# uoguelph-mlrg/Theano-MPI

Hardware: NVIDIA H100
Metric: AlexNet-128b BSP seconds per 5120 images (train+comm, device-timed, max over ranks) (lower is better)
Workload: dtype bf16; 1 GPU; model=AlexNet, global_batch=128, input=3x227x227, parallelism=dp1, rule=BSP, push_master=False, cuda_graph=True, overlap=True

## Files before the change

### theanompi_b200/csrc/api.h

```cpp
#pragma once
#include <cuda_runtime.h>
#include <stdint.h>
#include "common.cuh"

namespace tmpi {

constexpr int kMaxRanks = 8;
constexpr int kMaxCommBlocks = 1024;

struct CommCtx {
  void* arena[kMaxRanks];
  uint32_t* sig[kMaxRanks];
  uint32_t* epoch;
  void* mc_arena;
  int rank, world;
  long long spin_limit;
};

struct FusedArgs {
  CommCtx ctx;
  long long w_off, g_off, u_off, h_off, wire_off;
  const uint8_t* block_group;
  GroupTable tab;
  const float* lr_ptr;
  float mu;
// ... 2 lines not shown
  long long lo, hi;
  int wire16;
  int pre_reduced;
  int push_master = 1;
};

struct ReduceArgs {
  CommCtx ctx;
  long long src_off, dst_off, h_off;
  const uint8_t* block_group;
  GroupTable tab;
  float scale;
  long long lo, hi;
  int skip_local_groups;
};

void gemm_set_debug(int flags);
void gemm_set_bulk(int mask);
void gemm_rs_configure(int world, const void* const* peer_g , const void* local_g);
void gemm_rs_add_range(const void* c_lo, const void* c_hi, long long blo, long long per);
void gemm_rs_clear();
int gemm_plan_splits(int tiles, int num_kb, int sms);
int gemm_plan_tall(long long M, int nt, int out_bf16, int sms);
void gemm(const void* A, const void* B, void* C, const float* bias, int M, int N, int K, long long lda, long long ldb, long long ldc,
          int a_mn, int b_mn, int out_bf16, int bias_mode, int relu, float alpha, int bn_hint, int splitk, int f32, cudaStream_t st);
void gemm_sgd(const void* A, const void* B, void* W, void* U, void* H, const void* lr_ptr, float lr_mult, float wd, float mu, int nesterov,
              float inv_k, int M, int N, int K, long long lda, long long ldb, long long ldw, int f32, cudaStream_t st);

void conv_fprop(const void* x, const void* w, void* y, const float* bias, int N, int H, int W, int Ctot, int c_off, int Cg, int KH,
                int KW, int Ho, int Wo, int S, int P, int O, long long ldc, int relu, int dgrad, int f32, cudaStream_t st);
void conv_wgrad(const void* dy, const void* x, void* dw, int N, int H, int W, int Ctot, int c_off, int Cg, int KH, int KW, int Ho,
                int Wo, int S, int P, int O, long long ldy, int f32, cudaStream_t st);
void conv_fprop2(const void* x, const void* w0, const void* w1, void* y0, void* y1, const float* bias0, const float* bias1, int N, int H,
                 int W, int Ctot, int c_off0, int c_off1, int Cg, int KH, int KW, int Ho, int Wo, int S, int P, int O, long long ldc,
                 int relu, int dgrad, int f32, cudaStream_t st);
void conv_wgrad2(const void* dy0, const void* dy1, const void* x, void* dw0, void* dw1, int N, int H, int W, int Ctot, int c_off0,
                 int c_off1, int Cg, int KH, int KW, int Ho, int Wo, int S, int P, int O, long long ldy, int f32, cudaStream_t st);

void space_to_depth(const void* x, void* y, int N, int H, int W, int C, int S, int Hs, int Ws, int Cp, int P, int f32, cudaStream_t st);
void s2d_filter(const void* src, void* dst, int O, int KH, int KW, int C, int S, int KHs, int KWs, int Cp, int dir, int f32, cudaStream_t st);
void lrn_fwd(const void* x, void* y, long long rows, int C, int n, float k, float alpha, float beta, int f32, cudaStream_t st);
void lrn_bwd(const void* x, const void* dy, void* dx, long long rows, int C, int n, float k, float alpha, float beta, int f32, cudaStream_t st);
void pool_fwd(const void* x, void* y, void* arg, int N, int H, int W, int C, int Ho, int Wo, int k, int s, int p, int is_max, int f32,
              cudaStream_t st);
void pool_bwd(const void* dy, const void* arg, void* dx, int N, int H, int W, int C, int Ho, int Wo, int k, int s, int p, int is_max, int f32,
              cudaStream_t st);
// ... 75 lines not shown
```

### theanompi_b200/csrc/binding.cpp

```cpp
#include <pybind11/pybind11.h>
#include <pybind11/stl.h>

#include <cstring>
#include <memory>
#include <vector>

#include "api.h"
#include "peer_arena.h"

namespace py = pybind11;
using namespace tmpi;
typedef uintptr_t ptr_t;

static inline void* P(ptr_t p) { return reinterpret_cast<void*>(p); }
static inline cudaStream_t S(ptr_t s) { return reinterpret_cast<cudaStream_t>(s); }

static GroupTable make_table(const std::vector<float>& lr_mult, const std::vector<float>& wd, const std::vector<int>& exch) {
  GroupTable t;
  for (int i = 0; i < kMaxGroups; ++i) {
    t.lr_mult[i] = i < (int)lr_mult.size() ? lr_mult[i] : 1.f;
    t.wd[i] = i < (int)wd.size() ? wd[i] : 0.f;
    t.exch[i] = i < (int)exch.size() ? exch[i] : 1;
  }
  return t;
// ... 2 lines not shown
struct PyComm {
  std::unique_ptr<PeerArena> pa;
};

PYBIND11_MODULE(_tmpi_native, m) {
  m.doc() = "theanompi_b200 native sm_90a kernels and peer-memory runtime";
  m.def("launch_count", [] { return (unsigned long long)g_launch_count.load(); });
  m.def("reset_launch_count", [] { g_launch_count.store(0); });
  m.def("capture_status", [](ptr_t st) {
    cudaStreamCaptureStatus s = cudaStreamCaptureStatusNone;
    cudaError_t e = cudaStreamIsCapturing(S(st), &s);
    return py::make_tuple((int)e, (int)s);
  });
  m.attr("ARENA_BLOCK") = kArenaBlock;
  m.attr("MAX_RANKS") = kMaxRanks;
  m.attr("MAX_COMM_BLOCKS") = kMaxCommBlocks;

  m.def("gemm_set_debug", &gemm_set_debug);
  m.def("gemm_set_bulk", &gemm_set_bulk);
  m.def("gemm_rs_add_range", [](ptr_t c_lo, ptr_t c_hi, long long blo, long long per) { gemm_rs_add_range(P(c_lo), P(c_hi), blo, per); });
  m.def("gemm_rs_clear", &gemm_rs_clear);
  m.def("gemm_plan_splits", &gemm_plan_splits);
  m.def("gemm_plan_tall", &gemm_plan_tall);
  m.def("gemm", [](ptr_t A, ptr_t B, ptr_t C, ptr_t bias, int M, int N, int K, long long lda, long long ldb, long long ldc, int a_mn, int b_mn,
                   int out_bf16, int bias_mode, int relu, float alpha, int bn_hint, int splitk, int f32, ptr_t st) {
    gemm(P(A), P(B), P(C), (const float*)P(bias), M, N, K, lda, ldb, ldc, a_mn, b_mn, out_bf16, bias_mode, relu, alpha, bn_hint, splitk, f32,
         S(st));
  }, py::arg("A"), py::arg("B"), py::arg("C"), py::arg("bias"), py::arg("M"), py::arg("N"), py::arg("K"), py::arg("lda"), py::arg("ldb"),
     py::arg("ldc"), py::arg("a_mn"), py::arg("b_mn"), py::arg("out_bf16"), py::arg("bias_mode"), py::arg("relu"), py::arg("alpha"),
     py::arg("bn_hint"), py::arg("splitk"), py::arg("f32"), py::arg("st"));
  m.def("gemm_sgd", [](ptr_t A, ptr_t B, ptr_t W, ptr_t U, ptr_t H, ptr_t lr_ptr, float lr_mult, float wd, float mu, int nesterov, float inv_k,
                       int M, int N, int K, long long lda, long long ldb, long long ldw, int f32, ptr_t st) {
    gemm_sgd(P(A), P(B), P(W), P(U), P(H), P(lr_ptr), lr_mult, wd, mu, nesterov, inv_k, M, N, K, lda, ldb, ldw, f32, S(st));
  }, py::arg("A"), py::arg("B"), py::arg("W"), py::arg("U"), py::arg("H"), py::arg("lr_ptr"), py::arg("lr_mult"), py::arg("wd"),
     py::arg("mu"), py::arg("nesterov"), py::arg("inv_k"), py::arg("M"), py::arg("N"), py::arg("K"), py::arg("lda"), py::arg("ldb"),
     py::arg("ldw"), py::arg("f32"), py::arg("st"));

  m.def("conv_fprop", [](ptr_t x, ptr_t w, ptr_t y, ptr_t bias, int N, int H, int W, int Ctot, int c_off, int Cg, int KH, int KW, int Ho, int Wo,
                         int Sd, int Pd, int O, long long ldc, int relu, int dgrad, int f32, ptr_t st) {
    conv_fprop(P(x), P(w), P(y), (const float*)P(bias), N, H, W, Ctot, c_off, Cg, KH, KW, Ho, Wo, Sd, Pd, O, ldc, relu, dgrad, f32, S(st)); });
  m.def("conv_wgrad", [](ptr_t dy, ptr_t x, ptr_t dw, int N, int H, int W, int Ctot, int c_off, int Cg, int KH, int KW, int Ho, int Wo, int Sd,
                         int Pd, int O, long long ldy, int f32, ptr_t st) {
    conv_wgrad(P(dy), P(x), P(dw), N, H, W, Ctot, c_off, Cg, KH, KW, Ho, Wo, Sd, Pd, O, ldy, f32, S(st)); });
  m.def("conv_fprop2", [](ptr_t x, ptr_t w0, ptr_t w1, ptr_t y0, ptr_t y1, ptr_t b0, ptr_t b1, int N, int H, int W, int Ctot, int c_off0, int c_off1,
                          int Cg, int KH, int KW, int Ho, int Wo, int Sd, int Pd, int O, long long ldc, int relu, int dgrad, int f32, ptr_t st) {
    conv_fprop2(P(x), P(w0), P(w1), P(y0), P(y1), (const float*)P(b0), (const float*)P(b1), N, H, W, Ctot, c_off0, c_off1, Cg, KH, KW, Ho, Wo,
// ... 165 lines not shown
```

### theanompi_b200/csrc/gemm_wgmma.cu

```cuda
#include "gemm_wgmma.cuh"
#include <vector>

namespace tmpi {
std::atomic<unsigned long long> g_launch_count{0};

namespace wgmma {

int g_dbg = 0;
int g_bulk = -1;

static int choose_splits(int tiles, int num_kb, int sms) {
  if (deterministic_mode()) return 1;
  if (tiles >= sms || num_kb < 8) return 1;
  const int kTileOverheadKb = 4;
  int best = 1;
  long long best_cost = -1;
  const int max_s = std::min(num_kb / 4, 4 * sms);
  for (int s = 1; s <= max_s; ++s) {
    const int kb_per = (num_kb + s - 1) / s;
    const int s_eff = (num_kb + kb_per - 1) / kb_per;
    const long long waves = ((long long)tiles * s_eff + sms - 1) / sms;
    const long long cost = waves * (kb_per + kTileOverheadKb) * 64 + s_eff;
    if (best_cost < 0 || cost < best_cost) { best_cost = cost; best = s_eff; }
  }
  return best;
}

static bool use_tall_tiles(long long M, int nt, int eligible, int sms) {
  static const bool enabled = [] { const char* e = getenv("TMPI_GEMM_TALL"); return !(e && e[0] == '0'); }();
  if (!enabled || !eligible || M < 2 * BM) return false;
  const long long t1 = ((M + BM - 1) / BM) * nt, t2 = ((M + 2 * BM - 1) / (2 * BM)) * nt;
  const long long w1 = (t1 + sms - 1) / sms, w2 = (t2 + sms - 1) / sms;
  return w2 * 17 <= w1 * 10;
}

}

void gemm_set_debug(int flags) { wgmma::g_dbg = flags; }
void gemm_set_bulk(int mask) { wgmma::g_bulk = mask; }

namespace wgmma {
struct RsRange { const char* lo; const char* hi; long long blo, per; };
static int g_rs_world = 0, g_rs_rank = 0;
static float* g_rs_peer[kMaxRanks] = {};
static const char* g_rs_local = nullptr;
static std::vector<RsRange> g_rs_ranges;
static std::mutex g_rs_mu;
static bool rs_lookup(const void* C, Params& p) {
  std::lock_guard<std::mutex> lk(g_rs_mu);
  if (g_rs_world < 2) return false;
  const char* c = reinterpret_cast<const char*>(C);
  for (const RsRange& r : g_rs_ranges) {
    if (c >= r.lo && c < r.hi) {
      p.rs_world = g_rs_world; p.rs_rank = g_rs_rank;
      p.rs_blo = (unsigned)r.blo; p.rs_per = (unsigned)std::max<long long>(1, r.per);
      p.rs_e0 = (long long)((c - g_rs_local) / 4);
// ... 8 lines not shown
void gemm_rs_configure(int world, const void* const* peer_g, const void* local_g) {
  std::lock_guard<std::mutex> lk(wgmma::g_rs_mu);
  if (world > kMaxRanks) throw std::runtime_error("gemm_rs_configure: too many ranks");
  wgmma::g_rs_world = world;
  wgmma::g_rs_local = reinterpret_cast<const char*>(local_g);
  wgmma::g_rs_rank = 0;
  for (int q = 0; q < world; ++q) {
    wgmma::g_rs_peer[q] = reinterpret_cast<float*>(const_cast<void*>(peer_g[q]));
    if (peer_g[q] == local_g) wgmma::g_rs_rank = q;
  }
  wgmma::g_rs_ranges.clear();
}
void gemm_rs_add_range(const void* c_lo, const void* c_hi, long long blo, long long per) {
  std::lock_guard<std::mutex> lk(wgmma::g_rs_mu);
  wgmma::g_rs_ranges.push_back({reinterpret_cast<const char*>(c_lo), reinterpret_cast<const char*>(c_hi), blo, per});
}
void gemm_rs_clear() {
  std::lock_guard<std::mutex> lk(wgmma::g_rs_mu);
  wgmma::g_rs_world = 0; wgmma::g_rs_ranges.clear();
}

int gemm_plan_splits(int tiles, int num_kb, int sms) { return wgmma::choose_splits(tiles, num_kb, sms); }
int gemm_plan_tall(long long M, int nt, int out_bf16, int sms) { return wgmma::use_tall_tiles(M, nt, out_bf16, sms) ? 1 : 0; }

namespace wgmma {
template <typename T>
static void gemm_host(const void* A, const void* B, void* C, const float* bias, int M, int N, int K, long long lda, long long ldb,
                      long long ldc, int a_mn, int b_mn, int out_bf16, int bias_mode, int relu, float alpha, int bn_hint, int splitk,
                      cudaStream_t st) {
  using E = Elem<T>;
  constexpr int BK = E::BK, ATOM = E::ATOM, ESZ = E::ESZ;
  if (M <= 0 || N <= 0 || K <= 0) return;
  const int sms = sm_count();
  const int mt = (M + BM - 1) / BM;
  const bool fused_epi = bias_mode != 0 || relu;
  const bool can_split = (!out_bf16) && !fused_epi;
  int BN = bn_hint;
  if (BN == 0) {
    BN = 128;
    if (!(can_split && splitk != 1)) {
      if (mt * ((N + 127) / 128) < sms && N >= 64) BN = 64;
      if (BN == 64 && mt * ((N + 63) / 64) < sms && !b_mn && N >= 32) BN = 32;
    } else if (N <= 64) {
      BN = 64;
    }
  }
// ... 99 lines not shown
  cuuint64_t dims[3] = {(cuuint64_t)Cg, (cuuint64_t)taps, (cuuint64_t)O};
  cuuint64_t strides[2] = {(cuuint64_t)Cg * esz, (cuuint64_t)taps * Cg * esz};
  cuuint32_t box[3] = {(cuuint32_t)box_c, 1u, (cuuint32_t)box_o};
  cuuint32_t estr[3] = {1u, 1u, 1u};
  CUresult r = get_encode()(&m, esz == 4 ? f32_map_type() : CU_TENSOR_MAP_DATA_TYPE_BFLOAT16, 3, const_cast<void*>(w), dims, strides,
                            box, estr, CU_TENSOR_MAP_INTERLEAVE_NONE, swz, CU_TENSOR_MAP_L2_PROMOTION_L2_256B,
                            CU_TENSOR_MAP_FLOAT_OOB_FILL_NONE);
  if (r != CUDA_SUCCESS) throw std::runtime_error("tmpi_native: cuTensorMapEncodeTiled(3D weights) failed, code " + std::to_string((int)r));
  if (cache.size() > 4096) cache.clear();
  cache[key] = m;
  return m;
}

template <typename T>
static void conv_fprop_groups(int ngroups, const void* x, const int* c_off, const void* const* w, void* const* y, const float* const* bias,
                              int N, int H, int W, int Ctot, int Cg, int KH, int KW, int Ho, int Wo, int S, int P, int O, long long ldc,
                              int relu, int out_bf16, int dgrad, cudaStream_t st) {
  using E = Elem<T>;
  constexpr int BK = E::BK, ATOM = E::ATOM, ESZ = E::ESZ;
  const long long M = (long long)N * Ho * Wo;
  if (M <= 0 || O <= 0) return;
  if (M >= (1LL << 31)) throw std::runtime_error("conv_fprop: too many output pixels");
  if (ESZ == 4) out_bf16 = 0;
  const int BN = O > 64 ? 128 : 64;
  Params p;
  p.C = y[0]; p.bias = bias[0]; p.alpha = 1.f; p.M = (int)M; p.N = O; p.K = KH * KW * Cg; p.ldc = ldc; p.a_mn = 0; p.b_mn = dgrad ? 1 : 0;
  p.groups = ngroups; p.C1 = ngroups > 1 ? y[1] : nullptr; p.bias1 = ngroups > 1 ? bias[1] : nullptr;
  p.out_bf16 = out_bf16; p.bias_mode = bias[0] ? 1 : 0; p.relu = relu; p.atomic_out = 0;
  if (ngroups > 1 && ((bias[0] == nullptr) != (bias[1] == nullptr))) throw std::runtime_error("conv_fprop: both groups need a bias or none");
  if (dgrad && (S != 1 || ((O * ESZ) % 16) != 0)) throw std::runtime_error("conv dgrad through the fprop kernel needs stride 1 and 16-byte channel rows");
  p.nt = (O + BN - 1) / BN; p.splits = 1;
  const bool tall = use_tall_tiles(M, p.nt * ngroups, ESZ == 2 ? out_bf16 : !dgrad, sm_count());
  p.mt = tall ? (int)((M + 2 * BM - 1) / (2 * BM)) : (int)((M + BM - 1) / BM);
  p.group_m = 0;
  p.conv_mode = 1; p.cHo = Ho; p.cWo = Wo; p.cS = S; p.cP = P; p.cKH = KH; p.cKW = KW; p.cCg = Cg; p.c_chunks = (Cg + BK - 1) / BK;
  p.num_kb = KH * KW * p.c_chunks; p.kb_per_split = p.num_kb;
  CUtensorMap ta[2], tb[2];
  for (int g = 0; g < ngroups; ++g) {
    ta[g] = make_im2col_map(x, N, H, W, Ctot, c_off[g], Cg, KH, KW, S, P, BM, ESZ, 0);
    tb[g] = dgrad ? make_weight_map(w[g], Cg, KH * KW, O, BK, ATOM, ESZ, 1) : make_weight_map(w[g], O, KH * KW, Cg, BN, BK, ESZ, 0);
  }
  const CUtensorMap* a1 = ngroups > 1 ? &ta[1] : nullptr;
  const CUtensorMap* b1 = ngroups > 1 ? &tb[1] : nullptr;
  if (tall) { if (BN == 128) launch<T, 128, 2>(ta[0], tb[0], p, 1, st, a1, b1); else launch<T, 64, 2>(ta[0], tb[0], p, 1, st, a1, b1); }
  else if (BN == 128) launch<T, 128, 1>(ta[0], tb[0], p, 1, st, a1, b1);
  else launch<T, 64, 1>(ta[0], tb[0], p, 1, st, a1, b1);
}

template <typename T>
static void conv_wgrad_groups(int ngroups, const void* const* dy, const void* x, void* const* dw, const int* c_off, int N, int H, int W,
                              int Ctot, int Cg, int KH, int KW, int Ho, int Wo, int S, int P, int O, long long ldy, cudaStream_t st) {
  using E = Elem<T>;
  constexpr int BK = E::BK, ATOM = E::ATOM, ESZ = E::ESZ;
  const long long M = (long long)N * Ho * Wo;
  if (M <= 0 || O <= 0) return;
  if (M >= (1LL << 31)) throw std::runtime_error("conv_wgrad: too many output pixels");
  const int sms = sm_count();
  const int BN = 128;
  Params p;
  p.C = dw[0]; p.bias = nullptr; p.alpha = 1.f; p.M = O; p.N = KH * KW * Cg; p.K = (int)M; p.ldc = (long long)KH * KW * Cg; p.a_mn = 1; p.b_mn = 1;
  p.groups = ngroups; p.C1 = ngroups > 1 ? dw[1] : nullptr; p.bias1 = nullptr;
  p.out_bf16 = 0; p.bias_mode = 0; p.relu = 0;
  p.group_m = 0;
  p.conv_mode = 2; p.cHo = Ho; p.cWo = Wo; p.cS = S; p.cP = P; p.cKH = KH; p.cKW = KW; p.cCg = Cg; p.c_chunks = (Cg + ATOM - 1) / ATOM;
  p.mt = (O + BM - 1) / BM; p.nt = (KH * KW * p.c_chunks + BN / ATOM - 1) / (BN / ATOM);
  p.num_kb = (int)((M + BK - 1) / BK);
  int splits = choose_splits(p.mt * p.nt * ngroups, p.num_kb, sms);
  p.kb_per_split = (p.num_kb + splits - 1) / splits;
  splits = (p.num_kb + p.kb_per_split - 1) / p.kb_per_split;
  p.splits = splits; p.atomic_out = splits > 1;
  CUtensorMap ta[2], tb[2];
  for (int g = 0; g < ngroups; ++g) {
    if (splits > 1) check_cuda(cudaMemsetAsync(dw[g], 0, (size_t)O * KH * KW * Cg * 4, st), "conv_wgrad memset");
    ta[g] = make_tmap(dy[g], (uint64_t)O, (uint64_t)M, (uint64_t)ldy * ESZ, (uint32_t)BK, ESZ, 1);
    tb[g] = make_im2col_map(x, N, H, W, Ctot, c_off[g], Cg, KH, KW, S, P, BK, ESZ, 1);
  }
  launch<T, 128, 1>(ta[0], tb[0], p, splits, st, ngroups > 1 ? &ta[1] : nullptr, ngroups > 1 ? &tb[1] : nullptr);
}
}

void conv_fprop(const void* x, const void* w, void* y, const float* bias, int N, int H, int W, int Ctot, int c_off, int Cg, int KH,
                int KW, int Ho, int Wo, int S, int P, int O, long long ldc, int relu, int dgrad, int f32, cudaStream_t st) {
  const void* ws[1] = {w}; void* ys[1] = {y}; const float* bs[1] = {bias};
  if (f32) wgmma::conv_fprop_groups<float>(1, x, &c_off, ws, ys, bs, N, H, W, Ctot, Cg, KH, KW, Ho, Wo, S, P, O, ldc, relu, 0, dgrad, st);
  else wgmma::conv_fprop_groups<__nv_bfloat16>(1, x, &c_off, ws, ys, bs, N, H, W, Ctot, Cg, KH, KW, Ho, Wo, S, P, O, ldc, relu, 1, dgrad, st);
}

void conv_fprop2(const void* x, const void* w0, const void* w1, void* y0, void* y1, const float* bias0, const float* bias1, int N, int H,
                 int W, int Ctot, int c_off0, int c_off1, int Cg, int KH, int KW, int Ho, int Wo, int S, int P, int O, long long ldc,
                 int relu, int dgrad, int f32, cudaStream_t st) {
  const int co[2] = {c_off0, c_off1}; const void* ws[2] = {w0, w1}; void* ys[2] = {y0, y1}; const float* bs[2] = {bias0, bias1};
  if (f32) wgmma::conv_fprop_groups<float>(2, x, co, ws, ys, bs, N, H, W, Ctot, Cg, KH, KW, Ho, Wo, S, P, O, ldc, relu, 0, dgrad, st);
  else wgmma::conv_fprop_groups<__nv_bfloat16>(2, x, co, ws, ys, bs, N, H, W, Ctot, Cg, KH, KW, Ho, Wo, S, P, O, ldc, relu, 1, dgrad, st);
}

void conv_wgrad(const void* dy, const void* x, void* dw, int N, int H, int W, int Ctot, int c_off, int Cg, int KH, int KW, int Ho,
                int Wo, int S, int P, int O, long long ldy, int f32, cudaStream_t st) {
  const void* dys[1] = {dy}; void* dws[1] = {dw};
  if (f32) wgmma::conv_wgrad_groups<float>(1, dys, x, dws, &c_off, N, H, W, Ctot, Cg, KH, KW, Ho, Wo, S, P, O, ldy, st);
  else wgmma::conv_wgrad_groups<__nv_bfloat16>(1, dys, x, dws, &c_off, N, H, W, Ctot, Cg, KH, KW, Ho, Wo, S, P, O, ldy, st);
// ... 11 lines not shown
```

### theanompi_b200/csrc/gemm_wgmma.cuh

```cuda
#pragma once
#include "common.cuh"
#include "api.h"
#include <cuda.h>
#include <algorithm>
#include <map>
#include <mutex>
#include <tuple>

namespace tmpi {

namespace wgmma {

constexpr int BM = 128;
constexpr int NUM_THREADS = 384;
constexpr int NUM_CONSUMER_WARPS = 8;
constexpr int PRODUCER_REGS = 40, CONSUMER_REGS = 232;

template <typename T> struct SgdEpilogue {};
template <typename OP> struct Operand { using Type = OP; static constexpr bool kSgd = false; };
template <typename T> struct Operand<SgdEpilogue<T>> { using Type = T; static constexpr bool kSgd = true; };

template <typename T> struct Elem {
  static constexpr int ESZ = (int)sizeof(T);
  static constexpr int BK = 128 / ESZ;
// ... 177 lines not shown
}

__device__ __forceinline__ void wgmma(float (&d)[16], uint64_t da, uint64_t db, uint32_t scale_d, WgTF32<32>) {
  asm volatile("{\n\t.reg .pred p;\n\tsetp.ne.b32 p, %18, 0;\n\t"
               "wgmma.mma_async.sync.aligned.m64n32k8.f32.tf32.tf32 {%0, %1, %2, %3, %4, %5, %6, %7, %8, %9, %10, %11, %12, %13, %14, %15}, %16, %17, p, 1, 1;\n\t}"
               : "+f"(d[0]), "+f"(d[1]), "+f"(d[2]), "+f"(d[3]), "+f"(d[4]), "+f"(d[5]), "+f"(d[6]), "+f"(d[7]), "+f"(d[8]), "+f"(d[9]), "+f"(d[10]), "+f"(d[11]), "+f"(d[12]), "+f"(d[13]), "+f"(d[14]), "+f"(d[15])
               : "l"(da), "l"(db), "r"(scale_d));
}

__device__ __forceinline__ void wgmma(float (&d)[32], uint64_t da, uint64_t db, uint32_t scale_d, WgTF32<64>) {
  asm volatile("{\n\t.reg .pred p;\n\tsetp.ne.b32 p, %34, 0;\n\t"
               "wgmma.mma_async.sync.aligned.m64n64k8.f32.tf32.tf32 {%0, %1, %2, %3, %4, %5, %6, %7, %8, %9, %10, %11, %12, %13, %14, %15, %16, %17, %18, %19, %20, %21, %22, %23, %24, %25, %26, %27, %28, %29, %30, %31}, %32, %33, p, 1, 1;\n\t}"
               : "+f"(d[0]), "+f"(d[1]), "+f"(d[2]), "+f"(d[3]), "+f"(d[4]), "+f"(d[5]), "+f"(d[6]), "+f"(d[7]), "+f"(d[8]), "+f"(d[9]), "+f"(d[10]), "+f"(d[11]), "+f"(d[12]), "+f"(d[13]), "+f"(d[14]), "+f"(d[15]), "+f"(d[16]), "+f"(d[17]), "+f"(d[18]), "+f"(d[19]), "+f"(d[20]), "+f"(d[21]), "+f"(d[22]), "+f"(d[23]), "+f"(d[24]), "+f"(d[25]), "+f"(d[26]), "+f"(d[27]), "+f"(d[28]), "+f"(d[29]), "+f"(d[30]), "+f"(d[31])
               : "l"(da), "l"(db), "r"(scale_d));
}

__device__ __forceinline__ void wgmma(float (&d)[64], uint64_t da, uint64_t db, uint32_t scale_d, WgTF32<128>) {
  asm volatile("{\n\t.reg .pred p;\n\tsetp.ne.b32 p, %66, 0;\n\t"
               "wgmma.mma_async.sync.aligned.m64n128k8.f32.tf32.tf32 {%0, %1, %2, %3, %4, %5, %6, %7, %8, %9, %10, %11, %12, %13, %14, %15, %16, %17, %18, %19, %20, %21, %22, %23, %24, %25, %26, %27, %28, %29, %30, %31, %32, %33, %34, %35, %36, %37, %38, %39, %40, %41, %42, %43, %44, %45, %46, %47, %48, %49, %50, %51, %52, %53, %54, %55, %56, %57, %58, %59, %60, %61, %62, %63}, %64, %65, p, 1, 1;\n\t}"
               : "+f"(d[0]), "+f"(d[1]), "+f"(d[2]), "+f"(d[3]), "+f"(d[4]), "+f"(d[5]), "+f"(d[6]), "+f"(d[7]), "+f"(d[8]), "+f"(d[9]), "+f"(d[10]), "+f"(d[11]), "+f"(d[12]), "+f"(d[13]), "+f"(d[14]), "+f"(d[15]), "+f"(d[16]), "+f"(d[17]), "+f"(d[18]), "+f"(d[19]), "+f"(d[20]), "+f"(d[21]), "+f"(d[22]), "+f"(d[23]), "+f"(d[24]), "+f"(d[25]), "+f"(d[26]), "+f"(d[27]), "+f"(d[28]), "+f"(d[29]), "+f"(d[30]), "+f"(d[31]), "+f"(d[32]), "+f"(d[33]), "+f"(d[34]), "+f"(d[35]), "+f"(d[36]), "+f"(d[37]), "+f"(d[38]), "+f"(d[39]), "+f"(d[40]), "+f"(d[41]), "+f"(d[42]), "+f"(d[43]), "+f"(d[44]), "+f"(d[45]), "+f"(d[46]), "+f"(d[47]), "+f"(d[48]), "+f"(d[49]), "+f"(d[50]), "+f"(d[51]), "+f"(d[52]), "+f"(d[53]), "+f"(d[54]), "+f"(d[55]), "+f"(d[56]), "+f"(d[57]), "+f"(d[58]), "+f"(d[59]), "+f"(d[60]), "+f"(d[61]), "+f"(d[62]), "+f"(d[63])
               : "l"(da), "l"(db), "r"(scale_d));
}

__device__ __forceinline__ uint64_t make_smem_desc(uint32_t smem_addr, uint32_t lbo_bytes, uint32_t sbo_bytes) {
  uint64_t d = 0;
  d |= (uint64_t)((smem_addr & 0x3FFFF) >> 4);
  d |= (uint64_t)((lbo_bytes >> 4) & 0x3FFF) << 16;
  d |= (uint64_t)((sbo_bytes >> 4) & 0x3FFF) << 32;
  d |= (uint64_t)1 << 62;
  return d;
}

template <typename T, int BN, int MT, int TA, int TB>
__device__ __forceinline__ void mma_kblock(float (&acc)[MT][BN / 2], uint64_t da, uint64_t db, uint32_t a_step, uint32_t b_step) {
  constexpr int STEPS = Elem<T>::BK / Elem<T>::MMA_K;
  constexpr uint64_t SUB = (uint64_t)(BM * 128) >> 4;
#pragma unroll
  for (int k = 0; k < STEPS; ++k) {
#pragma unroll
    for (int u = 0; u < MT; ++u) {
      if constexpr (Elem<T>::TF32) wgmma(acc[u], da + u * SUB + a_step * k, db + b_step * k, 1u, WgTF32<BN>{});
      else wgmma(acc[u], da + u * SUB + a_step * k, db + b_step * k, 1u, WgBF16<BN, TA, TB>{});
    }
  }
}

__device__ __forceinline__ void xpose_tf32(uint8_t* dst, const uint8_t* src, int rows, int tid) {
  for (int c = tid; c < rows * 8; c += 128) {
    const int k = c & 31, mn = (c >> 5) * 4;
    const int mi = mn & 31;
    const float4 v = *reinterpret_cast<const float4*>(src + (mn >> 5) * 4096 + k * 128 + ((((mi >> 2) ^ (k & 7))) << 4));
    const float e[4] = {v.x, v.y, v.z, v.w};
#pragma unroll
    for (int i = 0; i < 4; ++i) {
      const int r = mn + i;
      uint32_t t;
      asm("cvt.rna.tf32.f32 %0, %1;" : "=r"(t) : "f"(e[i]));
      *reinterpret_cast<uint32_t*>(dst + r * 128 + ((((k >> 2) ^ (r & 7))) << 4) + (k & 3) * 4) = t;
    }
  }
}

__device__ __forceinline__ void tile_mn(const Params& p, int rem, int& mti, int& nti) {
  if (p.group_m <= 0) { nti = rem / p.mt; mti = rem - nti * p.mt; return; }
  const int band_sz = p.group_m * p.nt;
  const int band = rem / band_sz, within = rem - band * band_sz;
  const int rows = min(p.group_m, p.mt - band * p.group_m);
// ... 171 lines not shown
  }

  asm volatile("setmaxnreg.inc.sync.aligned.u32 %0;" ::"n"(CONSUMER_REGS));
  const int cw = wg - 1;
  const int ctid = threadIdx.x & 127;
  const int wi = warp & 3;
  const bool skip_mma = (p.dbg & 4) != 0;
  const bool a_mn = p.a_mn != 0, b_mn = p.b_mn != 0;
  const bool xa = C::XPOSE && a_mn, xb = C::XPOSE && b_mn;
  const uint32_t xa_base = xpose_base + (uint32_t)cw * (C::XA_BYTES + C::B_BYTES), xb_base = xa_base + C::XA_BYTES;
  constexpr uint32_t kMnStep = (uint32_t)(MMA_K * 128) >> 4;
  const uint32_t a_step = (a_mn && !xa) ? kMnStep : 2u, b_step = (b_mn && !xb) ? kMnStep : 2u;
  const uint32_t a_lbo = (a_mn && !xa) ? (uint32_t)(BK * 128) : 16u, b_lbo = (b_mn && !xb) ? (uint32_t)(BK * 128) : 16u;
  const int mode = E::TF32 ? 0 : ((a_mn ? 1 : 0) | (b_mn ? 2 : 0));

  const int esz = p.out_bf16 ? 2 : 4;
  const uint32_t pitch = (uint32_t)(32 * esz + 16);
  uint8_t* const wstage = generic(staging_base) + (size_t)(cw * 4 + wi) * 16 * C::STAGING_ROW;
  const int vec_per_row = (32 * esz) / 16;
  const int rows_per_it = 32 / vec_per_row;
  const int lr = lane / vec_per_row, lv = lane % vec_per_row;
  const bool ld_ok = (((long long)p.ldc * esz) % 16) == 0;
  const int fr = lane >> 2, fc = 2 * (lane & 3);
  float acc[MT][BN / 2];
  int stage = 0; uint32_t phase = 0;
  for (int tile = blockIdx.x; tile < total_tiles; tile += gridDim.x) {
    const int grp = tile >= per_group ? 1 : 0;
    const int t2 = tile - grp * per_group;
    const int split = t2 / tiles_mn, rem = t2 - split * tiles_mn;
    int mti, nti;
    tile_mn(p, rem, mti, nti);
    const int m0 = mti * TM, n0 = nti * BN;
    const int kb0 = split * p.kb_per_split, kb1 = min(num_kb_total, kb0 + p.kb_per_split);
#pragma unroll
    for (int u = 0; u < MT; ++u)
#pragma unroll
      for (int i = 0; i < BN / 2; ++i) acc[u][i] = 0.f;
    for (int kb = kb0; kb < kb1; ++kb) {
      mbar_wait(full_bar(stage), phase);
      const uint32_t sa = smem_base + stage * C::STAGE_BYTES;
      uint32_t a_addr = sa + (uint32_t)cw * (64 * 128), b_addr = sa + C::A_BYTES;
      if constexpr (C::XPOSE) {
        if (xa || xb) {
          wg_bar(cw);
          if (xa) { xpose_tf32(generic(xa_base), generic(a_addr), 64, ctid); a_addr = xa_base; }
          if (xb) { xpose_tf32(generic(xb_base), generic(b_addr), BN, ctid); b_addr = xb_base; }
          fence_proxy_async();
          wg_bar(cw);
        }
      }
      if (!skip_mma) {
        const uint64_t da = make_smem_desc(a_addr, a_lbo, 1024u), db = make_smem_desc(b_addr, b_lbo, 1024u);
#pragma unroll
        for (int u = 0; u < MT; ++u) acc_fence(acc[u]);
        wgmma_fence();
        if (mode == 0) mma_kblock<T, BN, MT, 0, 0>(acc, da, db, a_step, b_step);
        else if (mode == 1) mma_kblock<T, BN, MT, 1, 0>(acc, da, db, a_step, b_step);
        else if (mode == 2) mma_kblock<T, BN, MT, 0, 1>(acc, da, db, a_step, b_step);
        else mma_kblock<T, BN, MT, 1, 1>(acc, da, db, a_step, b_step);
        wgmma_commit();
        wgmma_wait0();
#pragma unroll
        for (int u = 0; u < MT; ++u) acc_fence(acc[u]);
      }
      __syncwarp();
      if (lane == 0) mbar_arrive(empty_bar(stage));
      if (++stage == C::STAGES) { stage = 0; phase ^= 1u; }
    }

    if constexpr (SGD) {
      const Params::Sgd& s = p.sgd;
      const Hyper h{*s.lr_ptr, s.mu, s.inv_k, s.nesterov};
      const int mbase = m0 + 64 * cw + 16 * wi;
      if (mbase >= p.M) continue;
      constexpr int kPitch = 32 * 4 + 16;
      const int vr = lane >> 3, vc = lane & 7;
      float4 wb[2][4], ub[2][4];
      auto load_wu = [&](int c, float4 (&w)[4], float4 (&u)[4]) {
        const int nb = n0 + 32 * c;
        if (nb + 32 > p.N) return;
#pragma unroll
        for (int it = 0; it < 4; ++it) {
          const long long gm = (long long)mbase + 4 * it + vr;
          if (gm < p.M) {
            const long long e = gm * s.ldw + nb + 4 * vc;
            w[it] = *reinterpret_cast<const float4*>(s.W + e);
// ... 257 lines not shown
```

Measured before the change: 0.1235 s/5120img.

## Add cost-model conv tile selection with n96/n192 tiles and trimmed MMA k-steps

Adds a cost model that picks the conv fprop, dgrad and wgrad tile width (64/96/128/192), the tall-tile choice and the split-K count from wave counts, replacing the fixed BN rules. It adds m64n96 and m64n192 wgmma variants for bf16 and tf32. In the main loop it skips wgmma on zero-padded channel tails (fewer k-steps on the last channel chunk) and on fully out-of-range M sub-tiles. The goal is to cut padding waste and wave quantization in the AlexNet conv layers, at the cost of more template instantiations, higher register pressure for n192 tiles, and a heuristic that may misjudge some shapes.

Result: faster. 0.1173 s/5120img, median of 6 (-5.0%).

```diff
diff --git a/theanompi_b200/csrc/api.h b/theanompi_b200/csrc/api.h
--- a/theanompi_b200/csrc/api.h
+++ b/theanompi_b200/csrc/api.h
@@ -1,6 +1,7 @@
 #pragma once
 #include <cuda_runtime.h>
 #include <stdint.h>
+#include <tuple>
 #include "common.cuh"
 
 namespace tmpi {
@@ -49,6 +50,7 @@
 void gemm_rs_clear();
 int gemm_plan_splits(int tiles, int num_kb, int sms);
 int gemm_plan_tall(long long M, int nt, int out_bf16, int sms);
+std::tuple<int, int, int> gemm_plan_conv(int kind, long long M, int N, int groups, int num_kb, int tall_ok, int sms);
 void gemm(const void* A, const void* B, void* C, const float* bias, int M, int N, int K, long long lda, long long ldb, long long ldc,
           int a_mn, int b_mn, int out_bf16, int bias_mode, int relu, float alpha, int bn_hint, int splitk, int f32, cudaStream_t st);
 void gemm_sgd(const void* A, const void* B, void* W, void* U, void* H, const void* lr_ptr, float lr_mult, float wd, float mu, int nesterov,
diff --git a/theanompi_b200/csrc/binding.cpp b/theanompi_b200/csrc/binding.cpp
--- a/theanompi_b200/csrc/binding.cpp
+++ b/theanompi_b200/csrc/binding.cpp
@@ -48,6 +48,7 @@
   m.def("gemm_rs_clear", &gemm_rs_clear);
   m.def("gemm_plan_splits", &gemm_plan_splits);
   m.def("gemm_plan_tall", &gemm_plan_tall);
+  m.def("gemm_plan_conv", &gemm_plan_conv);
   m.def("gemm", [](ptr_t A, ptr_t B, ptr_t C, ptr_t bias, int M, int N, int K, long long lda, long long ldb, long long ldc, int a_mn, int b_mn,
                    int out_bf16, int bias_mode, int relu, float alpha, int bn_hint, int splitk, int f32, ptr_t st) {
     gemm(P(A), P(B), P(C), (const float*)P(bias), M, N, K, lda, ldb, ldc, a_mn, b_mn, out_bf16, bias_mode, relu, alpha, bn_hint, splitk, f32,
diff --git a/theanompi_b200/csrc/gemm_wgmma.cu b/theanompi_b200/csrc/gemm_wgmma.cu
--- a/theanompi_b200/csrc/gemm_wgmma.cu
+++ b/theanompi_b200/csrc/gemm_wgmma.cu
@@ -32,6 +32,31 @@
   const long long t1 = ((M + BM - 1) / BM) * nt, t2 = ((M + 2 * BM - 1) / (2 * BM)) * nt;
   const long long w1 = (t1 + sms - 1) / sms, w2 = (t2 + sms - 1) / sms;
   return w2 * 17 <= w1 * 10;
+}
+
+struct ConvTile { int bn, mt, splits; };
+static ConvTile choose_conv_tile(int kind, long long M, int N, int groups, int num_kb, int tall_ok, int sms) {
+  static const int kCand[7][2] = {{128, 2}, {128, 1}, {192, 1}, {96, 2}, {96, 1}, {64, 2}, {64, 1}};
+  const int kTileOverheadKb = 4, kKblockCols = 64;
+  const int kWideWgradMinKb = 1024;
+  ConvTile best{0, 0, 1};
+  long long best_cost = -1;
+  for (const auto& c : kCand) {
+    const int bn = c[0], mt = c[1];
+    if (bn == 96 && kind != 0) continue;
+    if (kind == 2 && (bn == 64 || mt == 2)) continue;
+    if (kind == 2 && bn == 192 && num_kb < kWideWgradMinKb) continue;
+    const int nt = (N + bn - 1) / bn;
+    if (mt == 2 && !use_tall_tiles(M, nt * groups, tall_ok, sms)) continue;
+    const long long tiles = ((M + mt * BM - 1) / (mt * BM)) * nt * groups;
+    int splits = kind == 2 ? choose_splits((int)tiles, num_kb, sms) : 1;
+    const int kb_per = (num_kb + splits - 1) / splits;
+    splits = (num_kb + kb_per - 1) / kb_per;
+    const long long waves = (tiles * splits + sms - 1) / sms;
+    const long long cost = waves * (kb_per + kTileOverheadKb) * (mt * bn + kKblockCols);
+    if (best_cost < 0 || cost < best_cost) { best_cost = cost; best = {bn, mt, splits}; }
+  }
+  return best;
 }
 
 }
@@ -86,6 +111,10 @@
 
 int gemm_plan_splits(int tiles, int num_kb, int sms) { return wgmma::choose_splits(tiles, num_kb, sms); }
 int gemm_plan_tall(long long M, int nt, int out_bf16, int sms) { return wgmma::use_tall_tiles(M, nt, out_bf16, sms) ? 1 : 0; }
+std::tuple<int, int, int> gemm_plan_conv(int kind, long long M, int N, int groups, int num_kb, int tall_ok, int sms) {
+  const wgmma::ConvTile t = wgmma::choose_conv_tile(kind, M, N, groups, num_kb, tall_ok, sms);
+  return {t.bn, t.mt, t.splits};
+}
 
 namespace wgmma {
 template <typename T>
@@ -231,7 +260,10 @@
   if (M <= 0 || O <= 0) return;
   if (M >= (1LL << 31)) throw std::runtime_error("conv_fprop: too many output pixels");
   if (ESZ == 4) out_bf16 = 0;
-  const int BN = O > 64 ? 128 : 64;
+  const int c_chunks = (Cg + BK - 1) / BK, num_kb = KH * KW * c_chunks;
+  const ConvTile tile = choose_conv_tile(dgrad ? 1 : 0, M, O, ngroups, num_kb, ESZ == 2 ? out_bf16 : !dgrad, sm_count());
+  const int BN = tile.bn;
+  const bool tall = tile.mt == 2;
   Params p;
   p.C = y[0]; p.bias = bias[0]; p.alpha = 1.f; p.M = (int)M; p.N = O; p.K = KH * KW * Cg; p.ldc = ldc; p.a_mn = 0; p.b_mn = dgrad ? 1 : 0;
   p.groups = ngroups; p.C1 = ngroups > 1 ? y[1] : nullptr; p.bias1 = ngroups > 1 ? bias[1] : nullptr;
@@ -239,11 +271,10 @@
   if (ngroups > 1 && ((bias[0] == nullptr) != (bias[1] == nullptr))) throw std::runtime_error("conv_fprop: both groups need a bias or none");
   if (dgrad && (S != 1 || ((O * ESZ) % 16) != 0)) throw std::runtime_error("conv dgrad through the fprop kernel needs stride 1 and 16-byte channel rows");
   p.nt = (O + BN - 1) / BN; p.splits = 1;
-  const bool tall = use_tall_tiles(M, p.nt * ngroups, ESZ == 2 ? out_bf16 : !dgrad, sm_count());
   p.mt = tall ? (int)((M + 2 * BM - 1) / (2 * BM)) : (int)((M + BM - 1) / BM);
   p.group_m = 0;
-  p.conv_mode = 1; p.cHo = Ho; p.cWo = Wo; p.cS = S; p.cP = P; p.cKH = KH; p.cKW = KW; p.cCg = Cg; p.c_chunks = (Cg + BK - 1) / BK;
-  p.num_kb = KH * KW * p.c_chunks; p.kb_per_split = p.num_kb;
+  p.conv_mode = 1; p.cHo = Ho; p.cWo = Wo; p.cS = S; p.cP = P; p.cKH = KH; p.cKW = KW; p.cCg = Cg; p.c_chunks = c_chunks;
+  p.num_kb = num_kb; p.kb_per_split = p.num_kb;
   CUtensorMap ta[2], tb[2];
   for (int g = 0; g < ngroups; ++g) {
     ta[g] = make_im2col_map(x, N, H, W, Ctot, c_off[g], Cg, KH, KW, S, P, BM, ESZ, 0);
@@ -251,8 +282,13 @@
   }
   const CUtensorMap* a1 = ngroups > 1 ? &ta[1] : nullptr;
   const CUtensorMap* b1 = ngroups > 1 ? &tb[1] : nullptr;
-  if (tall) { if (BN == 128) launch<T, 128, 2>(ta[0], tb[0], p, 1, st, a1, b1); else launch<T, 64, 2>(ta[0], tb[0], p, 1, st, a1, b1); }
+  if (tall) {
+    if (BN == 128) launch<T, 128, 2>(ta[0], tb[0], p, 1, st, a1, b1);
+    else if (BN == 96) launch<T, 96, 2>(ta[0], tb[0], p, 1, st, a1, b1);
+    else launch<T, 64, 2>(ta[0], tb[0], p, 1, st, a1, b1);
+  } else if (BN == 192) launch<T, 192, 1>(ta[0], tb[0], p, 1, st, a1, b1);
   else if (BN == 128) launch<T, 128, 1>(ta[0], tb[0], p, 1, st, a1, b1);
+  else if (BN == 96) launch<T, 96, 1>(ta[0], tb[0], p, 1, st, a1, b1);
   else launch<T, 64, 1>(ta[0], tb[0], p, 1, st, a1, b1);
 }
 
@@ -264,19 +300,19 @@
   const long long M = (long long)N * Ho * Wo;
   if (M <= 0 || O <= 0) return;
   if (M >= (1LL << 31)) throw std::runtime_error("conv_wgrad: too many output pixels");
-  const int sms = sm_count();
-  const int BN = 128;
+  const int c_chunks = (Cg + ATOM - 1) / ATOM, num_kb = (int)((M + BK - 1) / BK);
+  const ConvTile tile = choose_conv_tile(2, O, KH * KW * c_chunks * ATOM, ngroups, num_kb, 0, sm_count());
+  const int BN = tile.bn;
   Params p;
   p.C = dw[0]; p.bias = nullptr; p.alpha = 1.f; p.M = O; p.N = KH * KW * Cg; p.K = (int)M; p.ldc = (long long)KH * KW * Cg; p.a_mn = 1; p.b_mn = 1;
   p.groups = ngroups; p.C1 = ngroups > 1 ? dw[1] : nullptr; p.bias1 = nullptr;
   p.out_bf16 = 0; p.bias_mode = 0; p.relu = 0;
   p.group_m = 0;
-  p.conv_mode = 2; p.cHo = Ho; p.cWo = Wo; p.cS = S; p.cP = P; p.cKH = KH; p.cKW = KW; p.cCg = Cg; p.c_chunks = (Cg + ATOM - 1) / ATOM;
+  p.conv_mode = 2; p.cHo = Ho; p.cWo = Wo; p.cS = S; p.cP = P; p.cKH = KH; p.cKW = KW; p.cCg = Cg; p.c_chunks = c_chunks;
   p.mt = (O + BM - 1) / BM; p.nt = (KH * KW * p.c_chunks + BN / ATOM - 1) / (BN / ATOM);
-  p.num_kb = (int)((M + BK - 1) / BK);
-  int splits = choose_splits(p.mt * p.nt * ngroups, p.num_kb, sms);
+  p.num_kb = num_kb;
+  const int splits = tile.splits;
   p.kb_per_split = (p.num_kb + splits - 1) / splits;
-  splits = (p.num_kb + p.kb_per_split - 1) / p.kb_per_split;
   p.splits = splits; p.atomic_out = splits > 1;
   CUtensorMap ta[2], tb[2];
   for (int g = 0; g < ngroups; ++g) {
@@ -284,7 +320,10 @@
     ta[g] = make_tmap(dy[g], (uint64_t)O, (uint64_t)M, (uint64_t)ldy * ESZ, (uint32_t)BK, ESZ, 1);
     tb[g] = make_im2col_map(x, N, H, W, Ctot, c_off[g], Cg, KH, KW, S, P, BK, ESZ, 1);
   }
-  launch<T, 128, 1>(ta[0], tb[0], p, splits, st, ngroups > 1 ? &ta[1] : nullptr, ngroups > 1 ? &tb[1] : nullptr);
+  const CUtensorMap* a1 = ngroups > 1 ? &ta[1] : nullptr;
+  const CUtensorMap* b1 = ngroups > 1 ? &tb[1] : nullptr;
+  if (BN == 192) launch<T, 192, 1>(ta[0], tb[0], p, splits, st, a1, b1);
+  else launch<T, 128, 1>(ta[0], tb[0], p, splits, st, a1, b1);
 }
 }
 
diff --git a/theanompi_b200/csrc/gemm_wgmma.cuh b/theanompi_b200/csrc/gemm_wgmma.cuh
--- a/theanompi_b200/csrc/gemm_wgmma.cuh
+++ b/theanompi_b200/csrc/gemm_wgmma.cuh
@@ -223,6 +223,36 @@
                : "l"(da), "l"(db), "r"(scale_d));
 }
 
+template <int TA, int TB>
+__device__ __forceinline__ void wgmma(float (&d)[48], uint64_t da, uint64_t db, uint32_t scale_d, WgBF16<96, TA, TB>) {
+  asm volatile("{\n\t.reg .pred p;\n\tsetp.ne.b32 p, %50, 0;\n\t"
+               "wgmma.mma_async.sync.aligned.m64n96k16.f32.bf16.bf16 {%0, %1, %2, %3, %4, %5, %6, %7, %8, %9, %10, %11, %12, %13, %14, %15, %16, %17, %18, %19, %20, %21, %22, %23, %24, %25, %26, %27, %28, %29, %30, %31, %32, %33, %34, %35, %36, %37, %38, %39, %40, %41, %42, %43, %44, %45, %46, %47}, %48, %49, p, 1, 1, %51, %52;\n\t}"
+               : "+f"(d[0]), "+f"(d[1]), "+f"(d[2]), "+f"(d[3]), "+f"(d[4]), "+f"(d[5]), "+f"(d[6]), "+f"(d[7]), "+f"(d[8]), "+f"(d[9]), "+f"(d[10]), "+f"(d[11]), "+f"(d[12]), "+f"(d[13]), "+f"(d[14]), "+f"(d[15]), "+f"(d[16]), "+f"(d[17]), "+f"(d[18]), "+f"(d[19]), "+f"(d[20]), "+f"(d[21]), "+f"(d[22]), "+f"(d[23]), "+f"(d[24]), "+f"(d[25]), "+f"(d[26]), "+f"(d[27]), "+f"(d[28]), "+f"(d[29]), "+f"(d[30]), "+f"(d[31]), "+f"(d[32]), "+f"(d[33]), "+f"(d[34]), "+f"(d[35]), "+f"(d[36]), "+f"(d[37]), "+f"(d[38]), "+f"(d[39]), "+f"(d[40]), "+f"(d[41]), "+f"(d[42]), "+f"(d[43]), "+f"(d[44]), "+f"(d[45]), "+f"(d[46]), "+f"(d[47])
+               : "l"(da), "l"(db), "r"(scale_d), "n"(TA), "n"(TB));
+}
+
+template <int TA, int TB>
+__device__ __forceinline__ void wgmma(float (&d)[96], uint64_t da, uint64_t db, uint32_t scale_d, WgBF16<192, TA, TB>) {
+  asm volatile("{\n\t.reg .pred p;\n\tsetp.ne.b32 p, %98, 0;\n\t"
+               "wgmma.mma_async.sync.aligned.m64n192k16.f32.bf16.bf16 {%0, %1, %2, %3, %4, %5, %6, %7, %8, %9, %10, %11, %12, %13, %14, %15, %16, %17, %18, %19, %20, %21, %22, %23, %24, %25, %26, %27, %28, %29, %30, %31, %32, %33, %34, %35, %36, %37, %38, %39, %40, %41, %42, %43, %44, %45, %46, %47, %48, %49, %50, %51, %52, %53, %54, %55, %56, %57, %58, %59, %60, %61, %62, %63, %64, %65, %66, %67, %68, %69, %70, %71, %72, %73, %74, %75, %76, %77, %78, %79, %80, %81, %82, %83, %84, %85, %86, %87, %88, %89, %90, %91, %92, %93, %94, %95}, %96, %97, p, 1, 1, %99, %100;\n\t}"
+               : "+f"(d[0]), "+f"(d[1]), "+f"(d[2]), "+f"(d[3]), "+f"(d[4]), "+f"(d[5]), "+f"(d[6]), "+f"(d[7]), "+f"(d[8]), "+f"(d[9]), "+f"(d[10]), "+f"(d[11]), "+f"(d[12]), "+f"(d[13]), "+f"(d[14]), "+f"(d[15]), "+f"(d[16]), "+f"(d[17]), "+f"(d[18]), "+f"(d[19]), "+f"(d[20]), "+f"(d[21]), "+f"(d[22]), "+f"(d[23]), "+f"(d[24]), "+f"(d[25]), "+f"(d[26]), "+f"(d[27]), "+f"(d[28]), "+f"(d[29]), "+f"(d[30]), "+f"(d[31]), "+f"(d[32]), "+f"(d[33]), "+f"(d[34]), "+f"(d[35]), "+f"(d[36]), "+f"(d[37]), "+f"(d[38]), "+f"(d[39]), "+f"(d[40]), "+f"(d[41]), "+f"(d[42]), "+f"(d[43]), "+f"(d[44]), "+f"(d[45]), "+f"(d[46]), "+f"(d[47]), "+f"(d[48]), "+f"(d[49]), "+f"(d[50]), "+f"(d[51]), "+f"(d[52]), "+f"(d[53]), "+f"(d[54]), "+f"(d[55]), "+f"(d[56]), "+f"(d[57]), "+f"(d[58]), "+f"(d[59]), "+f"(d[60]), "+f"(d[61]), "+f"(d[62]), "+f"(d[63]), "+f"(d[64]), "+f"(d[65]), "+f"(d[66]), "+f"(d[67]), "+f"(d[68]), "+f"(d[69]), "+f"(d[70]), "+f"(d[71]), "+f"(d[72]), "+f"(d[73]), "+f"(d[74]), "+f"(d[75]), "+f"(d[76]), "+f"(d[77]), "+f"(d[78]), "+f"(d[79]), "+f"(d[80]), "+f"(d[81]), "+f"(d[82]), "+f"(d[83]), "+f"(d[84]), "+f"(d[85]), "+f"(d[86]), "+f"(d[87]), "+f"(d[88]), "+f"(d[89]), "+f"(d[90]), "+f"(d[91]), "+f"(d[92]), "+f"(d[93]), "+f"(d[94]), "+f"(d[95])
+               : "l"(da), "l"(db), "r"(scale_d), "n"(TA), "n"(TB));
+}
+
+__device__ __forceinline__ void wgmma(float (&d)[48], uint64_t da, uint64_t db, uint32_t scale_d, WgTF32<96>) {
+  asm volatile("{\n\t.reg .pred p;\n\tsetp.ne.b32 p, %50, 0;\n\t"
+               "wgmma.mma_async.sync.aligned.m64n96k8.f32.tf32.tf32 {%0, %1, %2, %3, %4, %5, %6, %7, %8, %9, %10, %11, %12, %13, %14, %15, %16, %17, %18, %19, %20, %21, %22, %23, %24, %25, %26, %27, %28, %29, %30, %31, %32, %33, %34, %35, %36, %37, %38, %39, %40, %41, %42, %43, %44, %45, %46, %47}, %48, %49, p, 1, 1;\n\t}"
+               : "+f"(d[0]), "+f"(d[1]), "+f"(d[2]), "+f"(d[3]), "+f"(d[4]), "+f"(d[5]), "+f"(d[6]), "+f"(d[7]), "+f"(d[8]), "+f"(d[9]), "+f"(d[10]), "+f"(d[11]), "+f"(d[12]), "+f"(d[13]), "+f"(d[14]), "+f"(d[15]), "+f"(d[16]), "+f"(d[17]), "+f"(d[18]), "+f"(d[19]), "+f"(d[20]), "+f"(d[21]), "+f"(d[22]), "+f"(d[23]), "+f"(d[24]), "+f"(d[25]), "+f"(d[26]), "+f"(d[27]), "+f"(d[28]), "+f"(d[29]), "+f"(d[30]), "+f"(d[31]), "+f"(d[32]), "+f"(d[33]), "+f"(d[34]), "+f"(d[35]), "+f"(d[36]), "+f"(d[37]), "+f"(d[38]), "+f"(d[39]), "+f"(d[40]), "+f"(d[41]), "+f"(d[42]), "+f"(d[43]), "+f"(d[44]), "+f"(d[45]), "+f"(d[46]), "+f"(d[47])
+               : "l"(da), "l"(db), "r"(scale_d));
+}
+
+__device__ __forceinline__ void wgmma(float (&d)[96], uint64_t da, uint64_t db, uint32_t scale_d, WgTF32<192>) {
+  asm volatile("{\n\t.reg .pred p;\n\tsetp.ne.b32 p, %98, 0;\n\t"
+               "wgmma.mma_async.sync.aligned.m64n192k8.f32.tf32.tf32 {%0, %1, %2, %3, %4, %5, %6, %7, %8, %9, %10, %11, %12, %13, %14, %15, %16, %17, %18, %19, %20, %21, %22, %23, %24, %25, %26, %27, %28, %29, %30, %31, %32, %33, %34, %35, %36, %37, %38, %39, %40, %41, %42, %43, %44, %45, %46, %47, %48, %49, %50, %51, %52, %53, %54, %55, %56, %57, %58, %59, %60, %61, %62, %63, %64, %65, %66, %67, %68, %69, %70, %71, %72, %73, %74, %75, %76, %77, %78, %79, %80, %81, %82, %83, %84, %85, %86, %87, %88, %89, %90, %91, %92, %93, %94, %95}, %96, %97, p, 1, 1;\n\t}"
+               : "+f"(d[0]), "+f"(d[1]), "+f"(d[2]), "+f"(d[3]), "+f"(d[4]), "+f"(d[5]), "+f"(d[6]), "+f"(d[7]), "+f"(d[8]), "+f"(d[9]), "+f"(d[10]), "+f"(d[11]), "+f"(d[12]), "+f"(d[13]), "+f"(d[14]), "+f"(d[15]), "+f"(d[16]), "+f"(d[17]), "+f"(d[18]), "+f"(d[19]), "+f"(d[20]), "+f"(d[21]), "+f"(d[22]), "+f"(d[23]), "+f"(d[24]), "+f"(d[25]), "+f"(d[26]), "+f"(d[27]), "+f"(d[28]), "+f"(d[29]), "+f"(d[30]), "+f"(d[31]), "+f"(d[32]), "+f"(d[33]), "+f"(d[34]), "+f"(d[35]), "+f"(d[36]), "+f"(d[37]), "+f"(d[38]), "+f"(d[39]), "+f"(d[40]), "+f"(d[41]), "+f"(d[42]), "+f"(d[43]), "+f"(d[44]), "+f"(d[45]), "+f"(d[46]), "+f"(d[47]), "+f"(d[48]), "+f"(d[49]), "+f"(d[50]), "+f"(d[51]), "+f"(d[52]), "+f"(d[53]), "+f"(d[54]), "+f"(d[55]), "+f"(d[56]), "+f"(d[57]), "+f"(d[58]), "+f"(d[59]), "+f"(d[60]), "+f"(d[61]), "+f"(d[62]), "+f"(d[63]), "+f"(d[64]), "+f"(d[65]), "+f"(d[66]), "+f"(d[67]), "+f"(d[68]), "+f"(d[69]), "+f"(d[70]), "+f"(d[71]), "+f"(d[72]), "+f"(d[73]), "+f"(d[74]), "+f"(d[75]), "+f"(d[76]), "+f"(d[77]), "+f"(d[78]), "+f"(d[79]), "+f"(d[80]), "+f"(d[81]), "+f"(d[82]), "+f"(d[83]), "+f"(d[84]), "+f"(d[85]), "+f"(d[86]), "+f"(d[87]), "+f"(d[88]), "+f"(d[89]), "+f"(d[90]), "+f"(d[91]), "+f"(d[92]), "+f"(d[93]), "+f"(d[94]), "+f"(d[95])
+               : "l"(da), "l"(db), "r"(scale_d));
+}
+
 __device__ __forceinline__ uint64_t make_smem_desc(uint32_t smem_addr, uint32_t lbo_bytes, uint32_t sbo_bytes) {
   uint64_t d = 0;
   d |= (uint64_t)((smem_addr & 0x3FFFF) >> 4);
@@ -232,18 +262,40 @@
   return d;
 }
 
-template <typename T, int BN, int MT, int TA, int TB>
+template <typename T, int BN, int MT, int TA, int TB, int STEPS, int LIVE>
 __device__ __forceinline__ void mma_kblock(float (&acc)[MT][BN / 2], uint64_t da, uint64_t db, uint32_t a_step, uint32_t b_step) {
-  constexpr int STEPS = Elem<T>::BK / Elem<T>::MMA_K;
   constexpr uint64_t SUB = (uint64_t)(BM * 128) >> 4;
 #pragma unroll
+  for (int u = 0; u < MT; ++u) acc_fence(acc[u]);
+  wgmma_fence();
+#pragma unroll
   for (int k = 0; k < STEPS; ++k) {
 #pragma unroll
-    for (int u = 0; u < MT; ++u) {
+    for (int u = 0; u < LIVE; ++u) {
       if constexpr (Elem<T>::TF32) wgmma(acc[u], da + u * SUB + a_step * k, db + b_step * k, 1u, WgTF32<BN>{});
       else wgmma(acc[u], da + u * SUB + a_step * k, db + b_step * k, 1u, WgBF16<BN, TA, TB>{});
     }
   }
+  wgmma_commit();
+  wgmma_wait0();
+#pragma unroll
+  for (int u = 0; u < MT; ++u) acc_fence(acc[u]);
+}
+
+template <typename T, int BN, int MT, int TA, int TB, int LIVE>
+__device__ __forceinline__ void mma_kblock_steps(float (&acc)[MT][BN / 2], uint64_t da, uint64_t db, uint32_t a_step, uint32_t b_step,
+                                                 int steps) {
+  static_assert(Elem<T>::BK / Elem<T>::MMA_K == 4, "k-steps per k-block");
+  if (steps == 4) mma_kblock<T, BN, MT, TA, TB, 4, LIVE>(acc, da, db, a_step, b_step);
+  else if (steps == 3) mma_kblock<T, BN, MT, TA, TB, 3, LIVE>(acc, da, db, a_step, b_step);
+  else if (steps == 2) mma_kblock<T, BN, MT, TA, TB, 2, LIVE>(acc, da, db, a_step, b_step);
+  else mma_kblock<T, BN, MT, TA, TB, 1, LIVE>(acc, da, db, a_step, b_step);
+}
+template <typename T, int BN, int MT, int TA, int TB>
+__device__ __forceinline__ void mma_kblock_trim(float (&acc)[MT][BN / 2], uint64_t da, uint64_t db, uint32_t a_step, uint32_t b_step,
+                                                int steps, int n_live) {
+  if (MT == 2 && n_live == 1) mma_kblock_steps<T, BN, MT, TA, TB, 1>(acc, da, db, a_step, b_step, steps);
+  else mma_kblock_steps<T, BN, MT, TA, TB, MT>(acc, da, db, a_step, b_step, steps);
 }
 
 __device__ __forceinline__ void xpose_tf32(uint8_t* dst, const uint8_t* src, int rows, int tid) {
@@ -461,6 +513,9 @@
   const int lr = lane / vec_per_row, lv = lane % vec_per_row;
   const bool ld_ok = (((long long)p.ldc * esz) % 16) == 0;
   const int fr = lane >> 2, fc = 2 * (lane & 3);
+  constexpr int STEPS = BK / MMA_K;
+  const int k_chunks = p.conv_mode == 1 ? p.c_chunks : 1;
+  const int tail_steps = p.conv_mode == 1 ? (p.cCg - (p.c_chunks - 1) * BK + MMA_K - 1) / MMA_K : STEPS;
   float acc[MT][BN / 2];
   int stage = 0; uint32_t phase = 0;
   for (int tile = blockIdx.x; tile < total_tiles; tile += gridDim.x) {
@@ -471,36 +526,37 @@
     tile_mn(p, rem, mti, nti);
     const int m0 = mti * TM, n0 = nti * BN;
     const int kb0 = split * p.kb_per_split, kb1 = min(num_kb_total, kb0 + p.kb_per_split);
+    int n_live = 0;
+#pragma unroll
+    for (int u = 0; u < MT; ++u) n_live += (m0 + u * BM + 64 * cw < p.M) ? 1 : 0;
+    int cc = kb0 % k_chunks;
 #pragma unroll
     for (int u = 0; u < MT; ++u)
 #pragma unroll
       for (int i = 0; i < BN / 2; ++i) acc[u][i] = 0.f;
     for (int kb = kb0; kb < kb1; ++kb) {
       mbar_wait(full_bar(stage), phase);
+      const int steps = cc == k_chunks - 1 ? tail_steps : STEPS;
+      if (++cc == k_chunks) cc = 0;
       const uint32_t sa = smem_base + stage * C::STAGE_BYTES;
       uint32_t a_addr = sa + (uint32_t)cw * (64 * 128), b_addr = sa + C::A_BYTES;
-      if constexpr (C::XPOSE) {
-        if (xa || xb) {
-          wg_bar(cw);
-          if (xa) { xpose_tf32(generic(xa_base), generic(a_addr), 64, ctid); a_addr = xa_base; }
-          if (xb) { xpose_tf32(generic(xb_base), generic(b_addr), BN, ctid); b_addr = xb_base; }
-          fence_proxy_async();
-          wg_bar(cw);
-        }
-      }
-      if (!skip_mma) {
-        const uint64_t da = make_smem_desc(a_addr, a_lbo, 1024u), db = make_smem_desc(b_addr, b_lbo, 1024u);
-#pragma unroll
-        for (int u = 0; u < MT; ++u) acc_fence(acc[u]);
-        wgmma_fence();
-        if (mode == 0) mma_kblock<T, BN, MT, 0, 0>(acc, da, db, a_step, b_step);
-        else if (mode == 1) mma_kblock<T, BN, MT, 1, 0>(acc, da, db, a_step, b_step);
-        else if (mode == 2) mma_kblock<T, BN, MT, 0, 1>(acc, da, db, a_step, b_step);
-        else mma_kblock<T, BN, MT, 1, 1>(acc, da, db, a_step, b_step);
-        wgmma_commit();
-        wgmma_wait0();
-#pragma unroll
-        for (int u = 0; u < MT; ++u) acc_fence(acc[u]);
+      if (n_live > 0) {
+        if constexpr (C::XPOSE) {
+          if (xa || xb) {
+            wg_bar(cw);
+            if (xa) { xpose_tf32(generic(xa_base), generic(a_addr), 64, ctid); a_addr = xa_base; }
+            if (xb) { xpose_tf32(generic(xb_base), generic(b_addr), BN, ctid); b_addr = xb_base; }
+            fence_proxy_async();
+            wg_bar(cw);
+          }
+        }
+        if (!skip_mma) {
+          const uint64_t da = make_smem_desc(a_addr, a_lbo, 1024u), db = make_smem_desc(b_addr, b_lbo, 1024u);
+          if (mode == 0) mma_kblock_trim<T, BN, MT, 0, 0>(acc, da, db, a_step, b_step, steps, n_live);
+          else if (mode == 1) mma_kblock_trim<T, BN, MT, 1, 0>(acc, da, db, a_step, b_step, steps, n_live);
+          else if (mode == 2) mma_kblock_trim<T, BN, MT, 0, 1>(acc, da, db, a_step, b_step, steps, n_live);
+          else mma_kblock_trim<T, BN, MT, 1, 1>(acc, da, db, a_step, b_step, steps, n_live);
+        }
       }
       __syncwarp();
       if (lane == 0) mbar_arrive(empty_bar(stage));
```
